# singforai/mini-marl

Hardware: AMD Instinct MI355X
Metric: agent-env-steps/sec (4096 envs x 8 agents per GPU, QMIX GRU-64 rollout step) (higher is better)
Workload: dtype f32 (agent forward: fp16x3-split MFMA emulating f32 products, f32 accumulate); 1 GPU; QMIX 8-agent gridworld rollout, 4096 envs/GPU, GRU-64 agents, chunk 10, PER; envs_per_gpu=4096, agents=8, obs_dim=47, f1=64, gru=64, chunk=10, per_capacity_chunks=65536, per_prefilled_chunks=65536, parallelism=env-shard x1

## Files before the change

mini-marl_amd/csrc/agent_fwd.hip:

```cpp
#include <algorithm>
#include <cstdlib>
#include <type_traits>

#include "common.h"
#include "env_dev.h"
#include "minimarl.h"
#include "qnet_geo.h"
#include "rollout_env.h"

namespace mm {

struct QFwdParams {
  mm_qfwd_io io;
  QnetGeo g;
  const float* packed;
  int E, N, D, A;
  int nblocks;
  int stagger;
  int dbg;
  int pad_;
};

__device__ __forceinline__ void load_frag(const float* __restrict__ base, int lane, float (&a)[16]) {
#pragma unroll
// ... 910 lines not shown
}

typedef _Float16 f16x8 __attribute__((ext_vector_type(8)));
typedef float f32x4 __attribute__((ext_vector_type(4)));
typedef float f32x2 __attribute__((ext_vector_type(2)));

__host__ __device__ __forceinline__ int kperm16(int j, int g) { return 16 * (j >> 2) + 4 * g + (j & 3); }

__device__ __forceinline__ f32x4 mfma16x16(const f16x8& a, const f16x8& b, f32x4 c) {
  return __builtin_amdgcn_mfma_f32_16x16x32_f16(a, b, c, 0, 0, 0);
}

struct KS {
  f16x8 h, l;
};
typedef _Float16 f16x2_ __attribute__((ext_vector_type(2)));
typedef float f32x2_ __attribute__((ext_vector_type(2)));
__device__ __forceinline__ void split8(const float (&x)[8], KS& t, int lo_pairs = 4) {
  uint32_t hw[4], lw[4];
#pragma unroll
  for (int j = 0; j < 4; ++j) {
    const f32x2_ v = {x[2 * j], x[2 * j + 1]};
    hw[j] = __builtin_bit_cast(uint32_t, __builtin_convertvector(v, f16x2_));
    uint32_t lo;
    if (j >= lo_pairs) {
      lw[j] = 0u;
    } else {
      asm("v_fma_mixlo_f16 %0, %1, -1.0, %2 op_sel_hi:[1,0,0]" : "=v"(lo) : "v"(hw[j]), "v"(v.x));
      asm("v_fma_mixhi_f16 %0, %1, -1.0, %2 op_sel:[1,0,0] op_sel_hi:[1,0,0]" : "+v"(lo) : "v"(hw[j]), "v"(v.y));
      lw[j] = lo;
    }
  }
  t.h = __builtin_bit_cast(f16x8, hw);
  t.l = __builtin_bit_cast(f16x8, lw);
}
__device__ __forceinline__ void split_pair(const f32x4& a, const f32x4& b, KS& t) {
  float x[8];
#pragma unroll
  for (int r = 0; r < 4; ++r) {
    x[r] = a[r];
    x[4 + r] = b[r];
  }
  split8(x, t);
}
__device__ __forceinline__ void mm16(const float* __restrict__ blk, int q, const KS& x, int lane, f32x4& acc) {
  const f16x8 ah = *reinterpret_cast<const f16x8*>(blk + (q * 2) * 256 + lane * 4);
  const f16x8 al = *reinterpret_cast<const f16x8*>(blk + (q * 2 + 1) * 256 + lane * 4);
  acc = mfma16x16(al, x.h, acc);
  acc = mfma16x16(ah, x.l, acc);
  acc = mfma16x16(ah, x.h, acc);
}
__device__ __forceinline__ void mm16_x16(const float* __restrict__ blk, int q, const KS& x, int lane, f32x4& acc) {
  const f16x8 ah = *reinterpret_cast<const f16x8*>(blk + (q * 2) * 256 + lane * 4);
  const f16x8 al = *reinterpret_cast<const f16x8*>(blk + (q * 2 + 1) * 256 + lane * 4);
  acc = mfma16x16(al, x.h, acc);
  acc = mfma16x16(ah, x.h, acc);
}
struct Frag {
  f16x8 h, l;
};
__device__ __forceinline__ Frag ldfrag(const float* __restrict__ blk, int q, int lane) {
  Frag f;
  f.h = *reinterpret_cast<const f16x8*>(blk + (q * 2) * 256 + lane * 4);
  f.l = *reinterpret_cast<const f16x8*>(blk + (q * 2 + 1) * 256 + lane * 4);
  return f;
}
__device__ __forceinline__ void mmf(const Frag& a, const KS& x, f32x4& acc) {
  acc = mfma16x16(a.l, x.h, acc);
  acc = mfma16x16(a.h, x.l, acc);
  acc = mfma16x16(a.h, x.h, acc);
}
__device__ __forceinline__ f32x4 bias4(const float* __restrict__ b, int t, int g) {
  return *reinterpret_cast<const f32x4*>(b + 16 * t + 4 * g);
}
__device__ __forceinline__ void load_obs_ks(const float* orow, int kb, int D, float (&x)[8]) {
  const int g = (threadIdx.x & 63) >> 4;
#pragma unroll
  for (int j = 0; j < 8; ++j) {
    const int k = kb * 32 + kperm16(j, g);
    x[j] = (orow && k < D) ? orow[k] : 0.0f;
  }
}

template <int AT>
__device__ __forceinline__ int q_epilogue16(const QFwdParams& p, int agent, int e, bool valid,
                                            const f32x4 (&qa)[AT], float eps, uint64_t ctr, int64_t out_off = 0,
                                            const uint64_t* rng_in = nullptr) {
  const int g = (threadIdx.x & 63) >> 4;
  const mm_qfwd_io& io = p.io;
  if (valid && io.q_out) {
    float* qrow = io.q_out + (int64_t)e * io.q_se + (int64_t)agent * io.q_sa;
#pragma unroll
    for (int t = 0; t < AT; ++t)
#pragma unroll
      for (int r = 0; r < 4; ++r) {
        const int row = 16 * t + 4 * g + r;
        if (row < p.A) qrow[row] = qa[t][r];
      }
  }
  if (io.mode == MM_Q_NONE) return 0;
  float best = -INFINITY;
  int bi = 0x7fffffff;
#pragma unroll
  for (int t = 0; t < AT; ++t)
#pragma unroll
    for (int r = 0; r < 4; ++r) {
      const int row = 16 * t + 4 * g + r;
      const float v = qa[t][r];
      if (row < p.A && (v > best || (v == best && row < bi))) {
        best = v;
        bi = row;
      }
    }
#pragma unroll
  for (int o = 16; o <= 32; o <<= 1) {
    const float ob = __shfl_xor(best, o);
    const int oi = __shfl_xor(bi, o);
    if (ob > best || (ob == best && oi < bi)) {
      best = ob;
      bi = oi;
    }
  }
  int act = bi;
  if (io.mode == MM_Q_ACT) {
    if (!io.u && !io.rand_act) {
      const bool ra_lane = (g & 1) != 0;
      const uint64_t sd = ra_lane ? io.seed ^ 0x5bd1e995ull : io.seed;
      const uint64_t r = rng_in ? rng_draw_inner(sd, ctr, *rng_in)
                                : rng_draw(sd, ctr, (uint64_t)e, ra_lane ? (uint64_t)agent : 0xFFFFFFFFull);
      const float uu = rng_uniform(r);
      const uint32_t Au = (uint32_t)p.A;
      const int ra = (int)rng_mod_small_u(r, Au, 0xFFFFFFFFu / Au, (0xFFFFFFFFu % Au + 1u) % Au);
      const float uo = __shfl_xor(uu, 16);
      const int rao = __shfl_xor(ra, 16);
      if ((ra_lane ? uo : uu) <= eps) act = ra_lane ? ra : rao;
    } else {
      float u;
      if (io.u) {
        u = valid ? io.u[e] : 1.0f;
      } else {
        u = rng_uniform(rng_draw(io.seed, ctr, (uint64_t)e, 0xFFFFFFFFull));
      }
      if (u <= eps) {
        if (io.rand_act) {
          act = valid ? io.rand_act[(int64_t)e * p.N + agent] : 0;
        } else {
          act = (int)(rng_draw(io.seed ^ 0x5bd1e995ull, ctr, (uint64_t)e, (uint64_t)agent) % (uint64_t)p.A);
        }
      }
    }
  } else if (io.mode == MM_Q_GATHER) {
    act = valid ? io.act_in[(int64_t)e * io.act_se + agent] : 0;
  }
  float mine = 0.0f;
#pragma unroll
  for (int t = 0; t < AT; ++t)
#pragma unroll
    for (int r = 0; r < 4; ++r)
      if (16 * t + 4 * g + r == act) mine = qa[t][r];
  mine += __shfl_xor(mine, 16);
  mine += __shfl_xor(mine, 32);
  const float qsel = (io.mode == MM_Q_MAX) ? best : mine;
  if (valid && g == 0) {
    const int64_t o = out_off + (int64_t)e * p.N + agent;
    if (io.act_out && io.mode == MM_Q_ACT) io.act_out[o] = act;
    if (io.qsel_out) io.qsel_out[o] = qsel;
  }
  return act;
}

template <int F1, int G, int H, int AB, class OL>
__device__ __forceinline__ int agent_q_fwd_body_h3(const QFwdParams& p, int agent, int e,
                                                    const float* __restrict__ W, const OL& ol,
                                                    float (&xn)[8], const f32x4 (&h0)[H / 16], float eps,
                                                    uint64_t ctr, int64_t out_off = 0, int x16_from_kb = 1 << 30,
                                                    f32x4 (*h1_keep)[H / 16] = nullptr, bool store_h = true,
                                                    const uint64_t* rng_in = nullptr) {
  using CG = QnetCGeo<F1, G, H, AB>;
  constexpr int T1 = F1 / 16, T2 = G / 16, TH = H / 16, AT = (AB * 32 + 15) / 16;
  constexpr int RB1 = F1 / 32, RB2 = G / 32, HB = H / 32;
  const int lane = threadIdx.x & 63;
  const int g = lane >> 4;
  const bool valid = e < p.E;
  const mm_qfwd_io& io = p.io;
  const int ATr = (p.A + 15) / 16;
  constexpr int NWB = (CG::off_b1 + 15359) / 15360;
  auto lds_opaque = [](const float* q) {
    auto l = (const __attribute__((address_space(3))) float*)q;
    asm volatile("" : "+v"(l));
    return (const float*)l;
  };
  const float* WL[NWB];
#pragma unroll
  for (int k = 0; k < NWB; ++k) WL[k] = lds_opaque(W + 15360 * k + lane * 4);
  const float* WBias = lds_opaque(W + CG::off_b1 + 4 * g);
  auto wblk = [&](int off) { return WL[off / 15360] + (off % 15360); };
  auto wbias = [&](int off, int t) { return *reinterpret_cast<const f32x4*>(WBias + (off - CG::off_b1) + 16 * t); };
  auto mmb = [&](int off, int q, const KS& x, f32x4& acc) {
    const f16x8 ah = *reinterpret_cast<const f16x8*>(wblk(off) + (q * 2) * 256);
    const f16x8 al = *reinterpret_cast<const f16x8*>(wblk(off) + (q * 2 + 1) * 256);
    acc = mfma16x16(al, x.h, acc);
    acc = mfma16x16(ah, x.l, acc);
    acc = mfma16x16(ah, x.h, acc);
  };
  auto frag = [&](int off, int q) {
    Frag f;
    f.h = *reinterpret_cast<const f16x8*>(wblk(off) + (q * 2) * 256);
    f.l = *reinterpret_cast<const f16x8*>(wblk(off) + (q * 2 + 1) * 256);
    return f;
  };

  f32x4 x1[T1];
#pragma unroll
  for (int t = 0; t < T1; ++t) x1[t] = wbias(CG::off_b1, t);
  for (int kb = 0; kb < p.g.KD; ++kb) {
    KS ob;
    split8(xn, ob, kb >= x16_from_kb ? 0 : (x16_from_kb == 1 ? 1 : 4));
    if (kb + 1 < p.g.KD) ol(kb + 1, xn);
    if (kb >= x16_from_kb) {
#pragma unroll
      for (int t = 0; t < T1; ++t)
        mm16_x16(W + CG::off_l1 + (int64_t)((t >> 1) * p.g.KD + kb) * 1024, t & 1, ob, lane, x1[t]);
    } else {
#pragma unroll
      for (int t = 0; t < T1; ++t)
        mm16(W + CG::off_l1 + (int64_t)((t >> 1) * p.g.KD + kb) * 1024, t & 1, ob, lane, x1[t]);
    }
  }
  KS x1s[RB1];
#pragma unroll
  for (int t = 0; t < T1; ++t)
#pragma unroll
    for (int r = 0; r < 4; ++r) x1[t][r] = relu_bits(x1[t][r]);
#pragma unroll
  for (int kb = 0; kb < RB1; ++kb) split_pair(x1[2 * kb], x1[2 * kb + 1], x1s[kb]);
  float* sv = (io.save && valid) ? io.save + ((int64_t)e * p.N + agent) * (F1 + G + 6 * H) : nullptr;
  if (sv) {
#pragma unroll
    for (int t = 0; t < T1; ++t)
#pragma unroll
      for (int r = 0; r < 4; ++r) sv[16 * t + 4 * g + r] = x1[t][r];
  }

  f32x4 x2[T2];
#pragma unroll
  for (int t = 0; t < T2; ++t) {
    x2[t] = wbias(CG::off_b2, t);
#pragma unroll
    for (int kb = 0; kb < RB1; ++kb) mmb(CG::off_l2 + ((t >> 1) * RB1 + kb) * 1024, t & 1, x1s[kb], x2[t]);
#pragma unroll
    for (int r = 0; r < 4; ++r) x2[t][r] = relu_bits(x2[t][r]);
    if (sv) {
#pragma unroll
      for (int r = 0; r < 4; ++r) sv[F1 + 16 * t + 4 * g + r] = x2[t][r];
    }
  }
  KS x2s[RB2];
#pragma unroll
  for (int kb = 0; kb < RB2; ++kb) split_pair(x2[2 * kb], x2[2 * kb + 1], x2s[kb]);

  KS h0s[HB];
#pragma unroll
  for (int kb = 0; kb < HB; ++kb) split_pair(h0[2 * kb], h0[2 * kb + 1], h0s[kb]);
  float* hop = (valid && io.h_out && store_h) ? io.h_out + (int64_t)e * io.hout_se + (int64_t)agent * io.hout_sa +
                                         (int64_t)(4 * g) * io.hout_sf
                                   : nullptr;
  f32x4 h1[TH];
#pragma unroll
  for (int t = 0; t < TH; ++t) {
    const int rb = t >> 1, q = t & 1;
    f32x4 ar = wbias(CG::off_brz, t);
    f32x4 az = wbias(CG::off_brz + H, t);
    f32x4 anx = wbias(CG::off_bin, t);
    f32x4 anh = wbias(CG::off_bhn, t);
    auto tri = [&](int base, int gstride, const KS& x, f32x4& a0, f32x4& a1, f32x4& a2) {
      const Frag f0 = frag(base, q);
      const Frag f1 = frag(base + gstride, q);
      const Frag f2 = frag(base + 2 * gstride, q);
      a0 = mfma16x16(f0.l, x.h, a0);
      a1 = mfma16x16(f1.l, x.h, a1);
      a2 = mfma16x16(f2.l, x.h, a2);
      a0 = mfma16x16(f0.h, x.l, a0);
      a1 = mfma16x16(f1.h, x.l, a1);
      a2 = mfma16x16(f2.h, x.l, a2);
      a0 = mfma16x16(f0.h, x.h, a0);
      a1 = mfma16x16(f1.h, x.h, a1);
      a2 = mfma16x16(f2.h, x.h, a2);
    };
#pragma unroll
    for (int kb = 0; kb < RB2; ++kb) tri(CG::off_ih + (rb * RB2 + kb) * 1024, HB * RB2 * 1024, x2s[kb], ar, az, anx);
#pragma unroll
    for (int kb = 0; kb < HB; ++kb) tri(CG::off_hh + (rb * HB + kb) * 1024, HB * HB * 1024, h0s[kb], ar, az, anh);
    float rrs[4], zs[4], ns[4];
#pragma unroll
    for (int rp = 0; rp < 4; rp += 2) {
      const f32x2 vr = {ar[rp], ar[rp + 1]}, vz = {az[rp], az[rp + 1]};
      const f32x2 vx = {anx[rp], anx[rp + 1]}, vh = {anh[rp], anh[rp + 1]}, v0 = {h0[t][rp], h0[t][rp + 1]};
      f32x2 er = vr * -1.4426950408889634f, ez = vz * -1.4426950408889634f;
      er.x = __builtin_amdgcn_exp2f(er.x);
      er.y = __builtin_amdgcn_exp2f(er.y);
      ez.x = __builtin_amdgcn_exp2f(ez.x);
      ez.y = __builtin_amdgcn_exp2f(ez.y);
      er = er + 1.0f;
      ez = ez + 1.0f;
      f32x2 rr, z;
      rr.x = __builtin_amdgcn_rcpf(er.x);
      rr.y = __builtin_amdgcn_rcpf(er.y);
      z.x = __builtin_amdgcn_rcpf(ez.x);
      z.y = __builtin_amdgcn_rcpf(ez.y);
      f32x2 en = (vx + rr * vh) * 2.8853900817779268f;
      en.x = __builtin_amdgcn_exp2f(en.x);
      en.y = __builtin_amdgcn_exp2f(en.y);
      en = en + 1.0f;
      f32x2 n;
      n.x = __builtin_amdgcn_rcpf(en.x);
      n.y = __builtin_amdgcn_rcpf(en.y);
      n = 1.0f - 2.0f * n;
      const f32x2 hn = n + z * (v0 - n);
      h1[t][rp] = hn.x;
      h1[t][rp + 1] = hn.y;
      rrs[rp] = rr.x;
      rrs[rp + 1] = rr.y;
      zs[rp] = z.x;
      zs[rp + 1] = z.y;
      ns[rp] = n.x;
      ns[rp + 1] = n.y;
    }
    if (sv) {
#pragma unroll
      for (int r = 0; r < 4; ++r) {
        float* o = sv + F1 + G + 16 * t + 4 * g + r;
        o[0] = h0[t][r];
        o[H] = rrs[r];
        o[2 * H] = zs[r];
        o[3 * H] = ns[r];
        o[4 * H] = anh[r];
        o[5 * H] = h1[t][r];
      }
    }
    if (hop) {
#pragma unroll
      for (int r = 0; r < 4; ++r) hop[(int64_t)(16 * t + r) * io.hout_sf] = h1[t][r];
    }
  }
  if (h1_keep) {
#pragma unroll
    for (int t = 0; t < TH; ++t) (*h1_keep)[t] = h1[t];
  }
  KS h1s[HB];
#pragma unroll
  for (int kb = 0; kb < HB; ++kb) split_pair(h1[2 * kb], h1[2 * kb + 1], h1s[kb]);

  f32x4 qa[AT];
#pragma unroll
  for (int t = 0; t < AT; ++t) {
    qa[t] = wbias(CG::off_bq, t);
    if (t < ATr) {
#pragma unroll
      for (int kb = 0; kb < HB; ++kb) mmb(CG::off_q + ((t >> 1) * HB + kb) * 1024, t & 1, h1s[kb], qa[t]);
    }
  }
  return q_epilogue16<AT>(p, agent, e, valid, qa, eps, ctr, out_off, rng_in);
}

__device__ __forceinline__ bool agent_range_guarded(const QFwdParams& p, int agent) {
  return reinterpret_cast<const int*>(p.packed + 2 * p.g.agent_stride * p.N)[agent] != 0;
}
__device__ __forceinline__ const float* agent_image_src(const QFwdParams& p, int agent, bool exact) {
  return p.packed + (exact ? 0 : (int64_t)p.N * p.g.agent_stride) + (int64_t)agent * p.g.agent_stride;
}
__device__ __forceinline__ void image_dma(const float* src, float* wsm, int nchunk, int first_wave, int n_waves) {
  const int wave = threadIdx.x >> 6, lane = threadIdx.x & 63;
  if (wave >= first_wave)
    for (int c = wave - first_wave; c < nchunk; c += n_waves) glds_dwordx4(src + c * 256 + lane * 4, wsm + c * 256);
}
template <int H>
__device__ __forceinline__ void load_h0(const mm_qfwd_io& io, int ec, int agent, int g, f32x4 (&h0)[H / 16]) {
  const float* hp = io.h_in + (int64_t)ec * io.hin_se + (int64_t)agent * io.hin_sa + (int64_t)(4 * g) * io.hin_sf;
#pragma unroll
  for (int t = 0; t < H / 16; ++t)
#pragma unroll
    for (int r = 0; r < 4; ++r) h0[t][r] = hp[(int64_t)(16 * t + r) * io.hin_sf];
}

template <int F1, int G, int H, int AB>
__global__ __launch_bounds__(1024, 1) void agent_q_fwd_h3_kernel(QFwdParams p0, QFwdParams p1) {
  extern __shared__ __attribute__((aligned(16))) float wsm[];
  const bool second = (int)blockIdx.x >= p0.nblocks;
  const QFwdParams* kargs = (const QFwdParams*)__builtin_amdgcn_kernarg_segment_ptr();
  static_assert(sizeof(QFwdParams) % 8 == 0, "kernarg layout");
  const QFwdParams& p = kargs[second ? 1 : 0];
  (void)p1;
  const int bid = second ? (int)blockIdx.x - p0.nblocks : (int)blockIdx.x;
  const int agent = bid % p.N, tile = bid / p.N;
  const int wave = threadIdx.x >> 6, lane = threadIdx.x & 63;
  if (agent_range_guarded(p, agent)) {
    const int e32 = tile * 256 + wave * 32 + (lane & 31);
    const float* src32 = agent_image_src(p, agent, true);
    const int nch = (int)(p.g.agent_stride >> 8);
    for (int c = wave; c < nch; c += 16) glds_dwordx4(src32 + c * 256 + lane * 4, wsm + c * 256);
    const float* orow32 = obs_row_ptr(p, agent, e32);
    float x32[16];
    load_obs_kblock(orow32, 0, p.D, x32);
    const bool zero_h = e32 >= p.E || (p.io.reset && p.io.reset[e32]);
    __syncthreads();
    if (wave < 8)
      agent_q_fwd_body<F1, G, H, AB>(p, agent, e32, wsm,
                                     [&](int kb, float (&x)[16]) { load_obs_kblock(orow32, kb, p.D, x); }, x32,
                                     zero_h);
    return;
  }
  const int e = tile * 256 + wave * 16 + (lane & 15);
  const int g = lane >> 4;
  const float* src = agent_image_src(p, agent, false);
  const int nchunk = (int)(p.g.agent_stride >> 8);
  for (int c = wave; c < nchunk; c += 16) glds_dwordx4(src + c * 256 + lane * 4, wsm + c * 256);
  const mm_qfwd_io& io = p.io;
  const int ec = min(e, p.E - 1);
  f32x4 h0[H / 16];
  if (io.h_in) {
    load_h0<H>(io, ec, agent, g, h0);
  } else {
#pragma unroll
    for (int t = 0; t < H / 16; ++t) h0[t] = f32x4{0.f, 0.f, 0.f, 0.f};
  }
  const bool reset = io.reset && io.reset[ec];
  const float* orow = obs_row_ptr(p, agent, e);
  float xn[8];
  load_obs_ks(orow, 0, p.D, xn);
  const float eps = (io.mode == MM_Q_ACT && io.eps_ptr) ? *io.eps_ptr : io.epsilon;
  const uint64_t ctr = (io.mode == MM_Q_ACT && io.counter_ptr) ? *io.counter_ptr : io.counter;
  if (e >= p.E || reset) {
#pragma unroll
    for (int t = 0; t < H / 16; ++t) h0[t] = f32x4{0.f, 0.f, 0.f, 0.f};
  }
  __syncthreads();
  if (wave >= 8)
    for (int i = 0; i < p.stagger; ++i) __builtin_amdgcn_s_sleep(8);
  agent_q_fwd_body_h3<F1, G, H, AB>(p, agent, e, wsm,
                                    [&](int kb, float (&x)[8]) { load_obs_ks(orow, kb, p.D, x); }, xn, h0, eps, ctr);
}

struct RollStep {
  EnvDev env;
  const int32_t* act;
// ... 348 lines not shown
  uint64_t ctr0, seq;
  float eps;
  int tile, agent, e0;
  bool second, writer;
};

template <int F1, int G, int H, int AB>
__device__ __forceinline__ ChunkCtx chunk_ctx(const QFwdParams* kargs) {
  const RollChunk& rc = *reinterpret_cast<const RollChunk*>(kargs + 2);
  const int nb = (int)gridDim.x, b = (int)blockIdx.x;
  const int lb = (nb % 8 == 0) ? (b % 8) * (nb / 8) + b / 8 : b;
  const int N = kargs[0].N;
  ChunkCtx cx;
  cx.tile = lb / (2 * N);
  const int role = lb % (2 * N);
  cx.second = role >= N;
  cx.agent = cx.second ? role - N : role;
  cx.writer = !cx.second && cx.agent == 0;
  cx.e0 = cx.tile * 256;
  const RollChunkLds lay = roll_chunk_lds(rc.env.R, rc.env.C, N);
  char* envl = reinterpret_cast<char*>(wsm_ptr()) + rc.lds_env;
  cx.stab = reinterpret_cast<float*>(envl + lay.stab);
  cx.sgrid = reinterpret_cast<uint32_t*>(envl + lay.sgrid);
  cx.spq = reinterpret_cast<uint16_t*>(envl + lay.spq);
  cx.ssa = reinterpret_cast<uint16_t*>(envl + lay.ssa);
  cx.sdone = reinterpret_cast<uint8_t*>(envl + lay.sdone);
  cx.shx = reinterpret_cast<uint8_t*>(envl + lay.shx);
  cx.sgrp = reinterpret_cast<uint32_t*>(envl + lay.sgrp);
  cx.ctr0 = *rc.counter;
  cx.seq = *rc.seq;
  cx.eps = cx.second ? *kargs[1].io.eps_ptr : 0.0f;
  return cx;
}

typedef __attribute__((address_space(3))) uint32_t lds_u32_t;
__device__ __forceinline__ void grp_arrive(uint32_t* ctr, int lane) {
  asm volatile("s_waitcnt lgkmcnt(0)" ::: "memory");
  if (lane == 0) __hip_atomic_fetch_add((lds_u32_t*)ctr, 1u, __ATOMIC_RELAXED, __HIP_MEMORY_SCOPE_WORKGROUP);
  asm volatile("" ::: "memory");
}
__device__ __forceinline__ void grp_wait(uint32_t* ctr, uint32_t target, uint32_t* err, int lane) {
  auto seen = [&]() {
    return __builtin_amdgcn_readfirstlane(
               __hip_atomic_load((lds_u32_t*)ctr, __ATOMIC_RELAXED, __HIP_MEMORY_SCOPE_WORKGROUP)) >= target;
  };
  if (!seen()) {
    const uint64_t tw = __builtin_amdgcn_s_memrealtime();
    while (true) {
      __builtin_amdgcn_s_sleep(1);
      if (seen()) break;
      if (__builtin_amdgcn_s_memrealtime() - tw > kHandoffTimeout) {
        if (lane == 0) atomicOr(err, 2u);
        break;
      }
    }
  }
  asm volatile("" ::: "memory");
}

#if MM_ROLL_DEBUG
#define MM_CSTAMP(k)                                                                                          \
  do {                                                                                                        \
    if (rc.trace && lane == 0 && i < 12 && second) {                                                          \
      const int gj = roll_group_of_wave(wave);                                                                \
      const int ws = wave == roll_group_dyn_wave(gj) ? 0 : (wave == 4 * gj + ((gj + 1) & 3) ? 1 : -1);         \
      const int64_t ix = (((((int64_t)cx.tile * N + agent) * 4 + gj) * 2 + ws) * 12 + i) * 4 + (k);           \
      if (ws >= 0 && ix < 60000) rc.trace[ix] = __builtin_amdgcn_s_memrealtime();                             \
    }                                                                                                         \
  } while (0)
#else
#define MM_CSTAMP(k) \
  do {               \
  } while (0)
#endif

template <int F1, int G, int H, int AB, bool EXACT>
__device__ __forceinline__ void roll_chunk_steps() {
  const QFwdParams* kargs0 = (const QFwdParams*)__builtin_amdgcn_kernarg_segment_ptr();
  const int nsteps = reinterpret_cast<const RollChunk*>(kargs0 + 2)->n;
  f32x4 hkeep[H / 16];
#pragma unroll
  for (int t = 0; t < H / 16; ++t) hkeep[t] = f32x4{0.f, 0.f, 0.f, 0.f};
  uint64_t rin = 0;
  if (!EXACT) {
    const ChunkCtx c0x = chunk_ctx<F1, G, H, AB>(kargs0);
    const int l0 = (int)threadIdx.x & 63;
    const int e_r = c0x.e0 + ((int)threadIdx.x >> 6) * 16 + (l0 & 15);
    rin = rng_inner((uint64_t)e_r, ((l0 >> 4) & 1) ? (uint64_t)c0x.agent : 0xFFFFFFFFull);
  }
  for (int i = 0; i < nsteps; ++i) {
  int tz = 0;
  asm volatile("" : "+s"(tz));
  const QFwdParams* kargs =
      (const QFwdParams*)((const __attribute__((address_space(4))) char*)__builtin_amdgcn_kernarg_segment_ptr() + tz);
  (void)kargs0;
  const int tx = (int)threadIdx.x + tz;
  const int wave = tx >> 6, lane = tx & 63;
  const ChunkCtx cx = chunk_ctx<F1, G, H, AB>(kargs);
  const QFwdParams& p = kargs[cx.second ? 1 : 0];
  const RollChunk& rc = *reinterpret_cast<const RollChunk*>(kargs + 2);
  const int CL = rc.CL;
  const EnvDev& ev = rc.env;
  const int N = p.N, D = p.D, R = ev.R, C = ev.C, E = p.E;
  const int64_t EN = (int64_t)E * N, nd = (int64_t)N * D;
  const mm_qfwd_io& io = p.io;
  const int tile = cx.tile, agent = cx.agent, e0 = cx.e0;
  const bool second = cx.second, writer = cx.writer;
  const int grp = roll_group_of_wave(wave);
  const bool dynw = EXACT ? tx < 256 : wave == roll_group_dyn_wave(grp);
  uint32_t* gc = cx.sgrp + kRollGroupCtrs * grp;
  const int le_d = EXACT ? tx : roll_group_env0(grp) + lane, de = e0 + le_d;
  const bool dvalid = dynw && de < E;
  uint32_t* rows = cx.sgrid + le_d * roll_gbw(R);
  const int le = wave * 16 + (lane & 15), e = e0 + le;
  const int l32 = wave * 32 + (lane & 31), e32 = e0 + l32;
    int c = rc.c0 + i, kset = rc.set0;
    uint32_t kcs = rc.c0 == 0 ? 1u : 0u;
    while (c >= CL) {
      c -= CL;
      kset = kset + 1 == rc.S ? 0 : kset + 1;
      ++kcs;
    }
    const int64_t* stg = rc.staging + (int64_t)kset * E;
    const int pos = rc.pos0 + i >= rc.RL ? rc.pos0 + i - rc.RL : rc.pos0 + i;
    const int posn = pos + 1 == rc.RL ? 0 : pos + 1;
    const uint64_t ctr = cx.ctr0 + (uint64_t)i;
    const int cur = i & 1, prv = cur ^ 1;
    MM_CSTAMP(0);
    if (!EXACT &&
        __builtin_amdgcn_readfirstlane(wave) == roll_group_dyn_wave(__builtin_amdgcn_readfirstlane(grp)))
      __builtin_amdgcn_s_setprio(3);
    uint32_t aq[2] = {0u, 0u};
    if (i > 0) {
      if constexpr (!EXACT) {
        if (dynw) {
          const int w0 = roll_group_word0(grp);
          const uint64_t* hs = rc.hx + ((int64_t)tile * rc.hxl + i) * N * 32 + w0;
          uint32_t* hl = reinterpret_cast<uint32_t*>(cx.shx) + w0;
          const uint32_t tag = (uint32_t)cx.seq + 1u;
          constexpr int NQ = (kRollMaxN * 8 + 63) / 64;
          const int nw = N * 8;
          int wo[NQ];
          uint32_t got = 0u;
#pragma unroll
          for (int q = 0; q < NQ; ++q) {
            const int ix = q * 64 + lane;
            wo[q] = (ix >> 3) * 32 + (ix & 7);
            if (ix >= nw) got |= 1u << q;
          }
          const uint32_t need = (1u << NQ) - 1u;
          const uint64_t tw = __builtin_amdgcn_s_memrealtime();
          while (true) {
            uint64_t w[NQ];
#pragma unroll
            for (int q = 0; q < NQ; ++q)
              if (!((got >> q) & 1u)) w[q] = __hip_atomic_load(hs + wo[q], __ATOMIC_RELAXED, __HIP_MEMORY_SCOPE_AGENT);
#pragma unroll
            for (int q = 0; q < NQ; ++q)
              if (!((got >> q) & 1u) && (uint32_t)(w[q] >> 32) == tag) {
                hl[wo[q]] = (uint32_t)w[q];
                got |= 1u << q;
              }
            if (__all(got == need)) break;
            __builtin_amdgcn_s_sleep(1);
            if (__builtin_amdgcn_s_memrealtime() - tw > kHandoffTimeout) {
              if (lane == 0) atomicOr(rc.err, 2u);
// ... 96 lines not shown
      const int st = (int)cx.ssa[le_d] + 1;
      int apples = cx.ssa[256 + le_d];
      float* rout = rc.rew + (int64_t)pos * EN + (int64_t)de * N;
#pragma unroll
      for (int k = 0; k < kRollMaxN; ++k) {
        if (k < N) {
          const uint32_t w = pq[0] & 0xFFFFu;
          const int a = (int)(aq[0] & 15u);
#pragma unroll
          for (int j = 0; j < kRollMaxN / 2 - 1; ++j) pq[j] = __builtin_amdgcn_alignbit(pq[j + 1], pq[j], 16);
          pq[kRollMaxN / 2 - 1] >>= 16;
          aq[0] = __builtin_amdgcn_alignbit(aq[1], aq[0], 4);
          aq[1] >>= 4;
          const RollMove mv = roll_agent_step(w, a, k, rows, R, C, ev.step_cost);
          apples -= mv.ate ? 1 : 0;
          cx.spq[le_d * N + k] = (uint16_t)mv.w;
          if (writer) rout[k] = mv.rew;
        }
      }
      const bool dn = st >= ev.max_steps || apples == 0;
      cx.ssa[le_d] = (uint16_t)st;
      cx.ssa[256 + le_d] = (uint16_t)apples;
      cx.sdone[cur * 256 + le_d] = dn ? 1 : 0;
      if (writer) {
        rc.done[(int64_t)pos * E + de] = dn ? 1 : 0;
        rc.cur_row[de] = dn ? -1 : myrow;
      }
    }
    if constexpr (EXACT) {
      __syncthreads();
    } else {
      if (dynw)
        grp_arrive(gc + 1, lane);
      else
        grp_wait(gc + 1, (uint32_t)i + 1u, rc.err, lane);
    }
    MM_CSTAMP(2);
    const int64_t off = (int64_t)(second ? posn : pos) * EN;
    const int64_t nxt_off = (int64_t)(c + 1) * nd;
    if constexpr (EXACT) {
      const int hh = lane >> 5;
      if (wave < 8) {
        const bool ok32 = e32 < E;
        const bool r32 = !second && ok32 && cx.sdone[prv * 256 + l32];
        const bool bd = second && ok32 && cx.sdone[cur * 256 + l32];
        float* dst = (!second && srow >= 0) ? rc.store_obs + srow * rc.row_stride + nxt_off + (int64_t)agent * D : nullptr;
        const int ls = ok32 ? l32 : 0;
        const int rc32 = cx.spq[ls * N + agent] & 0xFF;
        const uint64_t wd32 = roll_obs_word(cx.sgrid + ls * roll_gbw(R), R, rc32 >> 4, rc32 & 15);
        const float cr32 = cx.stab[rc32 >> 4], cc32 = cx.stab[R + (rc32 & 15)];
        auto ol32 = [&](int kb, float (&x)[16]) {
#pragma unroll
          for (int q = 0; q < 4; ++q) {
            const int f0 = kb * 32 + 8 * q + 4 * hh;
            roll_feat4(wd32, f0, cr32, cc32, x + 4 * q);
            if (bd || !ok32)
#pragma unroll
              for (int j = 0; j < 4; ++j) x[4 * q + j] = (ok32 && f0 + j < D) ? ev.reset_obs[agent * D + f0 + j] : 0.0f;
            if (dst) roll_store4(dst, f0, D, x + 4 * q);
          }
        };
        float x32[16];
        ol32(0, x32);
        const int a = agent_q_fwd_body<F1, G, H, AB>(p, agent, ok32 ? e32 : E, wsm_ptr() + tz, ol32, x32,
                                                     !ok32 || r32 || bd, true, cx.eps, ctr, off);
        if (second && hh == 0 && ok32) cx.shx[l32] = (uint8_t)a;
      }
    } else {
      const int ec = min(e, E - 1);
      const int g = lane >> 4;
      f32x4 h0[H / 16];
      if (i == 0) {
        load_h0<H>(io, ec, agent, g, h0);
      } else {
#pragma unroll
        for (int t = 0; t < H / 16; ++t) h0[t] = hkeep[t];
      }
      const bool rt = !second && e < E && cx.sdone[prv * 256 + le];
      const bool bd = second && e < E && cx.sdone[cur * 256 + le];
      if (e >= E || rt || bd) {
#pragma unroll
        for (int t = 0; t < H / 16; ++t) h0[t] = f32x4{0.f, 0.f, 0.f, 0.f};
      }
      float* dst = (!second && srow >= 0) ? rc.store_obs + srow * rc.row_stride + nxt_off + (int64_t)agent * D : nullptr;
      const int ls = e < E ? le : 0;
      const int rcw = cx.spq[ls * N + agent] & 0xFF;
      const uint64_t wd = roll_obs_word_g(cx.sgrid + ls * roll_gbw(R), R, rcw >> 4, rcw & 15, g);
      const float cr = cx.stab[rcw >> 4], cc = cx.stab[R + (rcw & 15)];
      grp_arrive(gc + 0, lane);
      auto ol = [&](int kb, float (&x)[8]) {
#pragma unroll
        for (int q = 0; q < 2; ++q) {
          const int f0 = kb * 32 + 16 * q + 4 * g;
          roll_feat4(wd, f0, cr, cc, x + 4 * q);
          if (bd || e >= E)
#pragma unroll
            for (int j = 0; j < 4; ++j) x[4 * q + j] = (e < E && f0 + j < D) ? ev.reset_obs[agent * D + f0 + j] : 0.0f;
          if (dst) roll_store4(dst, f0, D, x + 4 * q);
        }
      };
      float xn[8];
      ol(0, xn);
      switch (__builtin_amdgcn_readfirstlane((grp + i) & 3)) {
        case 0: __builtin_amdgcn_s_setprio(0); break;
        case 1: __builtin_amdgcn_s_setprio(1); break;
        case 2: __builtin_amdgcn_s_setprio(2); break;
        default: __builtin_amdgcn_s_setprio(3); break;
      }
      const int a = agent_q_fwd_body_h3<F1, G, H, AB>(p, agent, e, wsm_ptr() + tz, ol, xn, h0, cx.eps, ctr, off, 1,
                                                      &hkeep, i + 1 == nsteps, &rin);
      if (second && i + 1 < rc.n) {
        uint32_t v = ((uint32_t)a & 15u) << (4 * (lane & 7));
        v |= __shfl_xor(v, 1);
        v |= __shfl_xor(v, 2);
        v |= __shfl_xor(v, 4);
        if (lane == 0 || lane == 8) {
          uint64_t* hd = rc.hx + (((int64_t)tile * rc.hxl + i + 1) * N + agent) * 32 + wave * 2 + (lane >> 3);
          __hip_atomic_store(hd, ((uint64_t)((uint32_t)cx.seq + 1u) << 32) | v, __ATOMIC_RELAXED,
                             __HIP_MEMORY_SCOPE_AGENT);
        }
      }
    }
    MM_CSTAMP(3);
    if (EXACT && second && i + 1 < rc.n) {
      __syncthreads();
      if (wave == 0 && lane < 32) {
        const uint2 b = reinterpret_cast<const uint2*>(cx.shx)[lane];
        uint64_t* hd = rc.hx + (((int64_t)tile * rc.hxl + i + 1) * N + agent) * 32 + lane;
        __hip_atomic_store(hd, ((uint64_t)((uint32_t)cx.seq + 1u) << 32) | nib_pack4(b.x) | (nib_pack4(b.y) << 16),
                           __ATOMIC_RELAXED, __HIP_MEMORY_SCOPE_AGENT);
      }
    }
  }
  if constexpr (!EXACT) __syncthreads();
}

template <int F1, int G, int H, int AB>
__global__ __launch_bounds__(1024, 1) void rollout_chunk_kernel(QFwdParams p0, QFwdParams p1, RollChunk rc_) {
  float* wsm = wsm_ptr();
  const QFwdParams* kargs = (const QFwdParams*)__builtin_amdgcn_kernarg_segment_ptr();
  const RollChunk& rc = *reinterpret_cast<const RollChunk*>(kargs + 2);
  (void)p0;
  (void)p1;
  (void)rc_;
  const int N = kargs[0].N;
  const ChunkCtx cx = chunk_ctx<F1, G, H, AB>(kargs);
  const int nb = (int)gridDim.x;
  const QFwdParams& p = kargs[cx.second ? 1 : 0];
  const EnvDev& ev = rc.env;
  const int R = ev.R, C = ev.C, RC = R * C, E = p.E;
  const int agent = cx.agent, e0 = cx.e0;
  const bool exact = agent_range_guarded(p, agent);
  const int par = *rc.envpar;

  image_dma(agent_image_src(p, agent, exact), wsm, (int)(p.g.agent_stride >> 8), 0, 16);
  if (threadIdx.x >= 256 && threadIdx.x < 256 + R + C) {
    const int i = threadIdx.x - 256;
    cx.stab[i] = i < R ? ev.rtab[i] : ev.ctab[i - R];
  }
  const int le_d = threadIdx.x, de = e0 + le_d;
  const bool dvalid = threadIdx.x < 256 && de < E;
  if (dvalid) {
    const int32_t* pw = (par ? ev.pos_alt : ev.pos) + (int64_t)de * N;
    const uint4* gin = reinterpret_cast<const uint4*>((par ? ev.grid_alt : ev.grid) + (int64_t)de * RC);
    uint32_t* rows = cx.sgrid + le_d * roll_gbw(R);
    cx.ssa[le_d] = (uint16_t)(par ? ev.steps_alt : ev.steps)[de];
    cx.ssa[256 + le_d] = (uint16_t)(par ? ev.apples_alt : ev.apples)[de];
    for (int k = 0; k < N; ++k) cx.spq[le_d * N + k] = (uint16_t)pos16(pw[k]);
    roll_unpack_rows(gin, rows, R);
    cx.sdone[256 + le_d] = rc.done_prev[de];
    if (cx.writer) {
      int ks = rc.set0;
      for (int k = 0; k < rc.S && k * rc.CL < rc.c0 + rc.n; ++k) {
        roll_row_ok(rc.staging[(int64_t)ks * E + de], rc.n_rows, rc.err);
        ks = ks + 1 == rc.S ? 0 : ks + 1;
      }
    }
  } else if (threadIdx.x < 256) {
    cx.sdone[256 + le_d] = 0;
  }
  if (threadIdx.x >= 512 && threadIdx.x < 512 + kRollGroups * kRollGroupCtrs) cx.sgrp[threadIdx.x - 512] = 0u;
  __syncthreads();

#if MM_ROLL_DEBUG
  uint64_t* clk = (rc.trace && threadIdx.x == 0) ? rc.trace + 60000 + 4 * (int)blockIdx.x : nullptr;
  if (clk) {
    clk[0] = __builtin_amdgcn_s_memtime();
    clk[1] = __builtin_amdgcn_s_memrealtime();
  }
#endif
  if (exact)
    roll_chunk_steps<F1, G, H, AB, true>();
  else
    roll_chunk_steps<F1, G, H, AB, false>();
#if MM_ROLL_DEBUG
  if (clk) {
    clk[2] = __builtin_amdgcn_s_memtime();
    clk[3] = __builtin_amdgcn_s_memrealtime();
// ... 653 lines not shown
  rc = make_params(d, packed_b, io_b, n_envs, &p1);
  if (rc) return rc;
  RollStep rs;
  rs.env = env->d;
  rs.act = x->act;
  rs.store_obs = x->store_obs;
  rs.row_stride = x->row_stride;
  rs.next_off = (int64_t)x->slot * nd;
  rs.staging = x->staging;
  rs.cur_row = x->cur_row;
  rs.rew = x->rew;
  rs.done = x->done;
  rs.counter = x->counter;
  rs.td = TdFuse{};
  if (x->td_on) {
    MM_REQUIRE(x->td_rew && x->td_done && x->td_qsel && x->td_maxq && x->td_act && x->chunk_td && x->store_act &&
                   x->store_rew && x->store_done, "rollout_step: null TD argument");
    MM_REQUIRE(x->td_slot >= 0 && x->td_slot < x->chunk_len, "rollout_step: bad TD slot");
    rs.td = TdFuse{x->td_rew, x->td_done, x->td_qsel, x->td_maxq, x->td_act, x->chunk_td, x->store_act,
                   x->store_rew, x->store_done, x->staging, nullptr, x->gamma, x->td_slot, x->chunk_len, 1};
  }
  rs.par = x->state_in;
#if MM_ROLL_DEBUG
  rs.trace = debug_trace_buffer("MM_ROLL_TRACE");
#else
  rs.trace = nullptr;
#endif
  MM_REQUIRE(x->n_rows >= 1 && x->n_rows < (1ll << 40), "rollout_step: n_rows must be the chunk store's row count");
  rs.n_rows = x->n_rows;
  rs.err = reinterpret_cast<uint32_t*>(x->err);
  rs.begin = x->begin ? 1 : 0;
  rs.lds_env = (int)roll_region(env->d, p0.g);
  if (with_qnet_shape(d, &rc, [&](auto F1, auto G, auto H, auto AB) {
        return launch_roll<F1, G, H, AB>(p0, p1, rs, sm, s);
      }))
    return rc;
  set_error("rollout_step: unsupported (F1,G,H)");
  return MM_EINVAL;
}

size_t rollout_chunk_lds(const mm_env* env, const mm_qnet_dims* d, int64_t n_envs) {
  if (rollout_step_lds(env, d, n_envs) == 0) return 0;
  const EnvDev& ev = env->d;
  QnetGeo g;
  QnetOffsets o;
  if (qnet_geometry(d, &g, &o)) return 0;
  const size_t img = ((size_t)g.agent_stride * 4 + 15) & ~size_t(15);
  const size_t sm = img + (size_t)roll_chunk_lds(ev.R, ev.C, ev.N).total;
  if (sm > 160 * 1024) return 0;
  int dev = 0, cus = 0;
  if (hipGetDevice(&dev) != hipSuccess || hipDeviceGetAttribute(&cus, hipDeviceAttributeMultiprocessorCount, dev) !=
                                              hipSuccess) {
    (void)hipGetLastError();
    return 0;
  }
  const int64_t nb = 2 * (int64_t)ev.N * ((n_envs + 255) / 256);
  return nb <= cus ? sm : 0;
}

int rollout_chunk(mm_env* env, const mm_qnet_dims* d, const float* packed_t, const mm_qfwd_io* io_t,
                  const float* packed_b, const mm_qfwd_io* io_b, int64_t n_envs, const mm_rollout_chunk_io* x,
                  hipStream_t s) {
  MM_REQUIRE(env && d && x && io_t && io_b, "rollout_chunk: null argument");
  const size_t sm = rollout_chunk_lds(env, d, n_envs);
  MM_REQUIRE(sm > 0, "rollout_chunk: configuration not supported (mm_rollout_chunk_supported)");
  const EnvDev& ev = env->d;
  MM_REQUIRE(x->store_obs && x->staging && x->cur_row && x->act0 && x->done_prev && x->rew && x->done && x->counter &&
                 x->ctl && x->handoff, "rollout_chunk: null buffer");
  MM_REQUIRE(x->chunk_len >= 1 && x->chunk_len <= 4096 && x->c0 >= 0 && x->c0 < x->chunk_len && x->n_steps >= 1,
             "rollout_chunk: bad chunk position / step count");
  MM_REQUIRE(x->n_sets >= 1 && x->n_sets <= 64 && x->set0 >= 0 && x->set0 < x->n_sets &&
                 x->c0 + x->n_steps <= (int64_t)x->n_sets * x->chunk_len,
             "rollout_chunk: the launch's steps span more chunks than staging sets (%d)", x->n_sets);
  MM_REQUIRE(x->ring_len >= 2 && x->ring_pos >= 0 && x->ring_pos < x->ring_len && x->n_steps < x->ring_len,
             "rollout_chunk: the rings must hold the launch's steps plus the next step's actions (n_steps < ring_len)");
  MM_REQUIRE(x->handoff_len >= x->n_steps, "rollout_chunk: handoff_len < n_steps");
  MM_REQUIRE(x->n_rows >= 1 && x->n_rows < (1ll << 40), "rollout_chunk: n_rows must be the chunk store's row count");
  MM_REQUIRE(io_t->mode == MM_Q_MAX && io_b->mode == MM_Q_ACT, "rollout_chunk: target io must be MAX, behavior io ACT");
  MM_REQUIRE(io_t->h_in && io_b->h_in && io_t->h_in == io_t->h_out && io_b->h_in == io_b->h_out,
             "rollout_chunk: hidden states required, updated in place");
  MM_REQUIRE(io_b->eps_ptr && io_b->act_out && io_b->qsel_out && io_t->qsel_out,
             "rollout_chunk: behavior eps_ptr / act_out / qsel_out and target qsel_out required");
  MM_REQUIRE(io_b->reset == nullptr && io_t->reset == nullptr, "rollout_chunk: reset flags come from the env (pass NULL)");
  const int64_t nd = (int64_t)d->n_agents * d->obs_dim;
  MM_REQUIRE(x->row_stride >= (x->chunk_len + 1) * nd, "rollout_chunk: row stride too small");
  QFwdParams p0, p1;
  mm_qfwd_io i0 = *io_t, i1 = *io_b;
  i0.obs = i1.obs = ev.reset_obs;
  int rc = make_params(d, packed_t, &i0, n_envs, &p0);
  if (rc) return rc;
  rc = make_params(d, packed_b, &i1, n_envs, &p1);
  if (rc) return rc;
  const int tiles = (int)((n_envs + 255) / 256);
  p0.nblocks = p1.nblocks = tiles * d->n_agents;
  RollChunk r;
  r.env = ev;
  r.store_obs = x->store_obs;
  r.row_stride = x->row_stride;
  r.staging = x->staging;
  r.cur_row = x->cur_row;
  r.n_rows = x->n_rows;
  r.act0 = x->act0;
  r.done_prev = x->done_prev;
  r.rew = x->rew;
  r.done = x->done;
  r.counter = reinterpret_cast<uint64_t*>(x->counter);
  r.seq = reinterpret_cast<uint64_t*>(x->ctl);
  r.envpar = reinterpret_cast<int32_t*>(x->ctl + 1);
  r.ticket = reinterpret_cast<uint32_t*>(x->ctl + 2);
  r.hx = reinterpret_cast<uint64_t*>(x->handoff);
  r.err = reinterpret_cast<uint32_t*>(x->err);
#if MM_ROLL_DEBUG
  r.trace = debug_trace_buffer("MM_ROLL_TRACE");
#else
  r.trace = nullptr;
#endif
  r.c0 = x->c0;
  r.n = x->n_steps;
  r.CL = x->chunk_len;
  r.S = x->n_sets;
  r.set0 = x->set0;
  r.RL = x->ring_len;
  r.pos0 = x->ring_pos;
  r.hxl = x->handoff_len;
  QnetGeo g;
  QnetOffsets o;
  qnet_geometry(d, &g, &o);
  r.lds_env = (int)(((size_t)g.agent_stride * 4 + 15) & ~size_t(15));
  const int nb = 2 * tiles * d->n_agents;
  if (with_qnet_shape(d, &rc, [&](auto F1, auto G, auto H, auto AB) {
        return launch_chunk<F1, G, H, AB>(p0, p1, r, nb, sm, s);
      }))
    return rc;
  set_error("rollout_chunk: unsupported (F1,G,H)");
  return MM_EINVAL;
}

}
```

mini-marl_amd/csrc/common.h:

```cpp
#pragma once
#include <hip/hip_runtime.h>
#include <stdint.h>

#define MM_OK 0
#define MM_EINVAL (-22)
#define MM_EHIP (-5)
#define MM_ENOMEM (-12)

namespace mm {

void set_error(const char* fmt, ...);

typedef float f32x16 __attribute__((ext_vector_type(16)));

__host__ __device__ __forceinline__ int kperm(int s, int h) { return (s & 3) + 8 * (s >> 2) + 4 * h; }

__device__ __forceinline__ f32x16 mfma32(float a, float b, f32x16 c) {
  return __builtin_amdgcn_mfma_f32_32x32x2f32(a, b, c, 0, 0, 0);
}

__device__ __forceinline__ float sigmoidf_(float x) {
  return __builtin_amdgcn_rcpf(1.0f + __builtin_amdgcn_exp2f(x * -1.4426950408889634f));
}
__device__ __forceinline__ float tanhf_(float x) {
  return 1.0f - 2.0f * __builtin_amdgcn_rcpf(1.0f + __builtin_amdgcn_exp2f(x * 2.8853900817779268f));
}

__device__ __forceinline__ uint64_t mix64(uint64_t z) {
  z += 0x9E3779B97F4A7C15ull;
  z = (z ^ (z >> 30)) * 0xBF58476D1CE4E5B9ull;
  z = (z ^ (z >> 27)) * 0x94D049BB133111EBull;
  return z ^ (z >> 31);
}
__device__ __forceinline__ uint64_t rng_draw(uint64_t seed, uint64_t counter, uint64_t a, uint64_t b) {
  return mix64(seed ^ mix64(counter * 0xD1B54A32D192ED03ull ^ mix64(a * 0x8CB92BA72F3D8DD7ull + b)));
}
__device__ __forceinline__ uint64_t rng_inner(uint64_t a, uint64_t b) { return mix64(a * 0x8CB92BA72F3D8DD7ull + b); }
__device__ __forceinline__ uint64_t rng_draw_inner(uint64_t seed, uint64_t counter, uint64_t inner) {
  return mix64(seed ^ mix64(counter * 0xD1B54A32D192ED03ull ^ inner));
}
__device__ __forceinline__ uint32_t umod_small(uint32_t x, uint32_t m, uint32_t minv) {
  uint32_t r = x - __umulhi(x, minv) * m;
  r = r >= m ? r - m : r;
  return r >= m ? r - m : r;
}
__device__ __forceinline__ float rollout_td(float sr, float sq, float st, float d, float gamma) {
  const float boot = __fmul_rn(__fmul_rn(1.0f - d, gamma), st);
  return fabsf(__fsub_rn(__fadd_rn(sr, boot), sq));
}
__device__ __forceinline__ float rng_uniform(uint64_t r) { return (float)(r >> 40) * (1.0f / 16777216.0f); }
__device__ __forceinline__ uint32_t rng_mod_small(uint64_t r, uint32_t m) {
  const uint32_t p32 = (0xFFFFFFFFu % m + 1u) % m;
  return ((uint32_t)(r >> 32) % m * p32 + (uint32_t)r % m) % m;
}
__device__ __forceinline__ uint32_t rng_mod_small_u(uint64_t r, uint32_t m, uint32_t minv, uint32_t p32) {
  return umod_small(umod_small((uint32_t)(r >> 32), m, minv) * p32 + umod_small((uint32_t)r, m, minv), m, minv);
}
__device__ __forceinline__ float relu_bits(float x) {
  return __int_as_float(max(__float_as_int(x), 0));
}

uint64_t* debug_trace_buffer(const char* env_name);

typedef __attribute__((address_space(3))) void lds_void_t;
__device__ __forceinline__ void glds_dword(const void* g, float* lds_base) {
  __builtin_amdgcn_global_load_lds(g, (lds_void_t*)lds_base, 4, 0, 0);
}
template <typename A>
__device__ __forceinline__ void glds_gather(float* dst, int n, A addr) {
  const int lane = threadIdx.x & 63, nw = blockDim.x >> 6;
  for (int c0 = (int)(threadIdx.x >> 6) * 64; c0 < n; c0 += nw * 64)
    if (c0 + lane < n) glds_dword(addr(c0 + lane), dst + c0);
}
template <typename A>
__device__ __forceinline__ void glds_rows(float* dst, int rows, int rowlen, int ld, A addr) {
  const int lane = threadIdx.x & 63, nw = blockDim.x >> 6;
  const int pr = (rowlen + 63) >> 6;
  for (int q = (int)(threadIdx.x >> 6); q < rows * pr; q += nw) {
    const int r = q / pr, c0 = (q - r * pr) * 64;
    if (c0 + lane < rowlen) glds_dword(addr(r, c0 + lane), dst + r * ld + c0);
  }
}

__device__ __forceinline__ void glds_dwordx4(const void* g, float* lds_base) {
  __builtin_amdgcn_global_load_lds(g, (lds_void_t*)lds_base, 16, 0, 0);
}
template <typename S>
__device__ __forceinline__ void glds_rows16(float* dst, int rows, int rowlen, int ld, S src) {
  const int lane = threadIdx.x & 63, nw = blockDim.x >> 6;
  const int pr = (rowlen + 255) >> 8;
  for (int q = (int)(threadIdx.x >> 6); q < rows * pr; q += nw) {
    const int r = q / pr, c0 = (q - r * pr) * 256;
    if (c0 + 4 * lane < rowlen) glds_dwordx4(src(r) + c0 + 4 * lane, dst + r * ld + c0);
  }
}

template <typename A>
__device__ __forceinline__ void glds16_gather(float* dst, int n4, A addr) {
  const int lane = threadIdx.x & 63, nw = blockDim.x >> 6;
  for (int c0 = (int)(threadIdx.x >> 6) * 64; c0 < n4; c0 += nw * 64)
    if (c0 + lane < n4) glds_dwordx4(addr(c0 + lane), dst + 4 * c0);
}

__device__ __forceinline__ void lds_sync() { asm volatile("s_waitcnt lgkmcnt(0)\n\ts_barrier" ::: "memory"); }

template <int K>
__device__ __forceinline__ float dot_seq(const float* w, const float* x, float acc) {
#pragma unroll
  for (int k = 0; k < K; ++k) acc += w[k] * x[k];
  return acc;
}
__device__ __forceinline__ float dot_seq_n(const float* w, const float* x, int K, float acc) {
  if (K == 64) return dot_seq<64>(w, x, acc);
  if (K == 32) return dot_seq<32>(w, x, acc);
  for (int k = 0; k < K; ++k) acc += w[k] * x[k];
  return acc;
}

struct TdFuse {
  const float* rew;
  const uint8_t* done;
  const float* q_taken;
// ... 41 lines not shown
```

Measured before the change: 1.714 billion agent-env-steps/s.

## Specialize chunk rollout step: carry split hidden state, single Q tile, lane-swap epilogue

Adds a compile-time StepChunk policy for the rollout chunk loop. It carries the already-split fp16 hidden state across steps instead of re-splitting h0, computes only one 16-row Q tile (n_actions <= 16), and drops the save/q_out paths. It also replaces the shuffle-based argmax and action reductions with permlane16/32 swaps and DPP, and batches RNG draws for two steps into one, carrying the decision to the odd step. This adds host-side requirements (n_actions <= 16, no q_out/save/u/rand_act) and changes which RNG lanes produce the draws, which may alter the random stream.

```diff
diff --git a/mini-marl_amd/csrc/agent_fwd.hip b/mini-marl_amd/csrc/agent_fwd.hip
--- a/mini-marl_amd/csrc/agent_fwd.hip
+++ b/mini-marl_amd/csrc/agent_fwd.hip
@@ -1016,10 +1016,100 @@
   }
 }
 
-template <int AT>
+struct StepGeneric {
+  static constexpr bool kGeneric = true;
+};
+struct StepChunk {
+  static constexpr bool kGeneric = false;
+};
+
+struct LanePair {
+  uint32_t lo, hi;
+};
+__device__ __forceinline__ LanePair lane_pair16(uint32_t v) {
+  const auto x = __builtin_amdgcn_permlane16_swap(v, v, false, false);
+  return LanePair{x[0], x[1]};
+}
+__device__ __forceinline__ LanePair lane_pair32(uint32_t v) {
+  const auto x = __builtin_amdgcn_permlane32_swap(v, v, false, false);
+  return LanePair{x[0], x[1]};
+}
+
+template <int MODE>
+__device__ __forceinline__ int q_epilogue16_chunk(const QFwdParams& p, int agent, int e, bool valid, const f32x4& q0,
+                                                  float eps, uint64_t ctr, int64_t out_off, const uint64_t* rng_in,
+                                                  bool odd_step, int& carry) {
+  const int g = (threadIdx.x & 63) >> 4;
+  const mm_qfwd_io& io = p.io;
+  float best = -INFINITY;
+  int bi = 0x7fffffff;
+#pragma unroll
+  for (int r = 0; r < 4; ++r) {
+    const int row = 4 * g + r;
+    const float v = q0[r];
+    if (row < p.A && (v > best || (v == best && row < bi))) {
+      best = v;
+      bi = row;
+    }
+  }
+  auto better = [&](const LanePair& v, const LanePair& ix) {
+    const float fa = __uint_as_float(v.lo), fb = __uint_as_float(v.hi);
+    const int ia = (int)ix.lo, ib = (int)ix.hi;
+    const bool tb = fb > fa || (fb == fa && ib < ia);
+    best = tb ? fb : fa;
+    bi = tb ? ib : ia;
+  };
+  better(lane_pair16(__float_as_uint(best)), lane_pair16((uint32_t)bi));
+  better(lane_pair32(__float_as_uint(best)), lane_pair32((uint32_t)bi));
+  static_assert(MODE == MM_Q_ACT || MODE == MM_Q_MAX, "chunk step epilogue: behavior (ACT) or target (MAX)");
+  if constexpr (MODE == MM_Q_MAX) {
+    if (valid && g == 0) io.qsel_out[out_off + (int64_t)e * p.N + agent] = best;
+    return bi;
+  } else {
+    int dec;
+    if (!odd_step) {
+      const bool ra_lane = (g & 1) != 0;
+      const uint64_t sd = ra_lane ? io.seed ^ 0x5bd1e995ull : io.seed;
+      const uint64_t r = rng_draw_premul(sd, (g & 2) ? rng_counter_mul(ctr + 1) : rng_counter_mul(ctr), *rng_in);
+      const float uu = rng_uniform(r);
+      const uint32_t Au = (uint32_t)p.A;
+      const uint32_t ra = rng_mod_small_u(r, Au, 0xFFFFFFFFu / Au, (0xFFFFFFFFu % Au + 1u) % Au);
+      const float u = __uint_as_float(lane_pair16(__float_as_uint(uu)).lo);
+      const int d = u <= eps ? (int)lane_pair16(ra).hi : -1;
+      const LanePair dd = lane_pair32((uint32_t)d);
+      dec = (int)dd.lo;
+      carry = (int)dd.hi;
+    } else {
+      dec = carry;
+    }
+    const int act = dec >= 0 ? dec : bi;
+    float mine = 0.0f;
+#pragma unroll
+    for (int r = 0; r < 4; ++r)
+      if (4 * g + r == act) mine = q0[r];
+    const LanePair m16 = lane_pair16(__float_as_uint(mine));
+    mine = __uint_as_float(m16.lo) + __uint_as_float(m16.hi);
+    const LanePair m32 = lane_pair32(__float_as_uint(mine));
+    mine = __uint_as_float(m32.lo) + __uint_as_float(m32.hi);
+    if (valid && g == 0) {
+      const int64_t o = out_off + (int64_t)e * p.N + agent;
+      io.act_out[o] = act;
+      io.qsel_out[o] = mine;
+    }
+    return act;
+  }
+}
+
+template <int AT, class POL = StepGeneric>
 __device__ __forceinline__ int q_epilogue16(const QFwdParams& p, int agent, int e, bool valid,
                                             const f32x4 (&qa)[AT], float eps, uint64_t ctr, int64_t out_off = 0,
-                                            const uint64_t* rng_in = nullptr) {
+                                            const uint64_t* rng_in = nullptr, bool odd_step = false,
+                                            int* carry = nullptr) {
+  if constexpr (!POL::kGeneric) {
+    if (p.io.mode == MM_Q_ACT)
+      return q_epilogue16_chunk<MM_Q_ACT>(p, agent, e, valid, qa[0], eps, ctr, out_off, rng_in, odd_step, *carry);
+    return q_epilogue16_chunk<MM_Q_MAX>(p, agent, e, valid, qa[0], eps, ctr, out_off, rng_in, odd_step, *carry);
+  }
   const int g = (threadIdx.x & 63) >> 4;
   const mm_qfwd_io& io = p.io;
   if (valid && io.q_out) {
@@ -1103,15 +1193,17 @@
   return act;
 }
 
-template <int F1, int G, int H, int AB, class OL>
+template <int F1, int G, int H, int AB, class OL, class POL = StepGeneric>
 __device__ __forceinline__ int agent_q_fwd_body_h3(const QFwdParams& p, int agent, int e,
                                                     const float* __restrict__ W, const OL& ol,
                                                     float (&xn)[8], const f32x4 (&h0)[H / 16], float eps,
                                                     uint64_t ctr, int64_t out_off = 0, int x16_from_kb = 1 << 30,
                                                     f32x4 (*h1_keep)[H / 16] = nullptr, bool store_h = true,
-                                                    const uint64_t* rng_in = nullptr) {
+                                                    const uint64_t* rng_in = nullptr, bool odd_step = false,
+                                                    int* carry = nullptr, KS (*hs_carry)[H / 32] = nullptr) {
   using CG = QnetCGeo<F1, G, H, AB>;
   constexpr int T1 = F1 / 16, T2 = G / 16, TH = H / 16, AT = (AB * 32 + 15) / 16;
+  constexpr int QT = POL::kGeneric ? AT : 1;
   constexpr int RB1 = F1 / 32, RB2 = G / 32, HB = H / 32;
   const int lane = threadIdx.x & 63;
   const int g = lane >> 4;
@@ -1168,7 +1260,9 @@
     for (int r = 0; r < 4; ++r) x1[t][r] = relu_bits(x1[t][r]);
 #pragma unroll
   for (int kb = 0; kb < RB1; ++kb) split_pair(x1[2 * kb], x1[2 * kb + 1], x1s[kb]);
-  float* sv = (io.save && valid) ? io.save + ((int64_t)e * p.N + agent) * (F1 + G + 6 * H) : nullptr;
+  float* sv = nullptr;
+  if constexpr (POL::kGeneric)
+    sv = (io.save && valid) ? io.save + ((int64_t)e * p.N + agent) * (F1 + G + 6 * H) : nullptr;
   if (sv) {
 #pragma unroll
     for (int t = 0; t < T1; ++t)
@@ -1194,11 +1288,16 @@
   for (int kb = 0; kb < RB2; ++kb) split_pair(x2[2 * kb], x2[2 * kb + 1], x2s[kb]);
 
   KS h0s[HB];
-#pragma unroll
-  for (int kb = 0; kb < HB; ++kb) split_pair(h0[2 * kb], h0[2 * kb + 1], h0s[kb]);
-  float* hop = (valid && io.h_out && store_h) ? io.h_out + (int64_t)e * io.hout_se + (int64_t)agent * io.hout_sa +
-                                         (int64_t)(4 * g) * io.hout_sf
-                                   : nullptr;
+  if constexpr (!POL::kGeneric) {
+#pragma unroll
+    for (int kb = 0; kb < HB; ++kb) h0s[kb] = (*hs_carry)[kb];
+  } else {
+#pragma unroll
+    for (int kb = 0; kb < HB; ++kb) split_pair(h0[2 * kb], h0[2 * kb + 1], h0s[kb]);
+  }
+  float* hop = (valid && (!POL::kGeneric || io.h_out) && store_h)
+                   ? io.h_out + (int64_t)e * io.hout_se + (int64_t)agent * io.hout_sa + (int64_t)(4 * g) * io.hout_sf
+                   : nullptr;
   f32x4 h1[TH];
 #pragma unroll
   for (int t = 0; t < TH; ++t) {
@@ -1284,17 +1383,21 @@
   KS h1s[HB];
 #pragma unroll
   for (int kb = 0; kb < HB; ++kb) split_pair(h1[2 * kb], h1[2 * kb + 1], h1s[kb]);
-
-  f32x4 qa[AT];
-#pragma unroll
-  for (int t = 0; t < AT; ++t) {
+  if constexpr (!POL::kGeneric) {
+#pragma unroll
+    for (int kb = 0; kb < HB; ++kb) (*hs_carry)[kb] = h1s[kb];
+  }
+
+  f32x4 qa[QT];
+#pragma unroll
+  for (int t = 0; t < QT; ++t) {
     qa[t] = wbias(CG::off_bq, t);
-    if (t < ATr) {
+    if (!POL::kGeneric || t < ATr) {
 #pragma unroll
       for (int kb = 0; kb < HB; ++kb) mmb(CG::off_q + ((t >> 1) * HB + kb) * 1024, t & 1, h1s[kb], qa[t]);
     }
   }
-  return q_epilogue16<AT>(p, agent, e, valid, qa, eps, ctr, out_off, rng_in);
+  return q_epilogue16<QT, POL>(p, agent, e, valid, qa, eps, ctr, out_off, rng_in, odd_step, carry);
 }
 
 __device__ __forceinline__ bool agent_range_guarded(const QFwdParams& p, int agent) {
@@ -1809,6 +1912,8 @@
 #pragma unroll
   for (int t = 0; t < H / 16; ++t) hkeep[t] = f32x4{0.f, 0.f, 0.f, 0.f};
   uint64_t rin = 0;
+  KS hsk[H / 32] = {};
+  int dcarry = -1;
   if (!EXACT) {
     const ChunkCtx c0x = chunk_ctx<F1, G, H, AB>(kargs0);
     const int l0 = (int)threadIdx.x & 63;
@@ -2071,6 +2176,13 @@
 #pragma unroll
         for (int t = 0; t < H / 16; ++t) h0[t] = f32x4{0.f, 0.f, 0.f, 0.f};
       }
+      if (i == 0) {
+#pragma unroll
+        for (int kb = 0; kb < H / 32; ++kb) split_pair(h0[2 * kb], h0[2 * kb + 1], hsk[kb]);
+      } else if (e >= E || rt || bd) {
+#pragma unroll
+        for (int kb = 0; kb < H / 32; ++kb) hsk[kb] = KS{};
+      }
       float* dst = (!second && srow >= 0) ? rc.store_obs + srow * rc.row_stride + nxt_off + (int64_t)agent * D : nullptr;
       const int ls = e < E ? le : 0;
       const int rcw = cx.spq[ls * N + agent] & 0xFF;
@@ -2096,13 +2208,14 @@
         case 2: __builtin_amdgcn_s_setprio(2); break;
         default: __builtin_amdgcn_s_setprio(3); break;
       }
-      const int a = agent_q_fwd_body_h3<F1, G, H, AB>(p, agent, e, wsm_ptr() + tz, ol, xn, h0, cx.eps, ctr, off, 1,
-                                                      &hkeep, i + 1 == nsteps, &rin);
+      const int a = agent_q_fwd_body_h3<F1, G, H, AB, decltype(ol), StepChunk>(
+          p, agent, e, wsm_ptr() + tz, ol, xn, h0, cx.eps, ctr, off, 1, &hkeep, i + 1 == nsteps, &rin, (i & 1) != 0,
+          &dcarry, &hsk);
       if (second && i + 1 < rc.n) {
         uint32_t v = ((uint32_t)a & 15u) << (4 * (lane & 7));
-        v |= __shfl_xor(v, 1);
-        v |= __shfl_xor(v, 2);
-        v |= __shfl_xor(v, 4);
+        v |= (uint32_t)__builtin_amdgcn_update_dpp(0, (int)v, 0xB1, 0xF, 0xF, false);
+        v |= (uint32_t)__builtin_amdgcn_update_dpp(0, (int)v, 0x4E, 0xF, 0xF, false);
+        v |= (uint32_t)__builtin_amdgcn_update_dpp(0, (int)v, 0x141, 0xF, 0xF, false);
         if (lane == 0 || lane == 8) {
           uint64_t* hd = rc.hx + (((int64_t)tile * rc.hxl + i + 1) * N + agent) * 32 + wave * 2 + (lane >> 3);
           __hip_atomic_store(hd, ((uint64_t)((uint32_t)cx.seq + 1u) << 32) | v, __ATOMIC_RELAXED,
@@ -2922,6 +3035,9 @@
   MM_REQUIRE(io_b->eps_ptr && io_b->act_out && io_b->qsel_out && io_t->qsel_out,
              "rollout_chunk: behavior eps_ptr / act_out / qsel_out and target qsel_out required");
   MM_REQUIRE(io_b->reset == nullptr && io_t->reset == nullptr, "rollout_chunk: reset flags come from the env (pass NULL)");
+  MM_REQUIRE(d->n_actions <= 16, "rollout_chunk: the hand-off words carry 4-bit actions (n_actions <= 16)");
+  MM_REQUIRE(!io_b->u && !io_b->rand_act && !io_b->save && !io_t->save && !io_b->q_out && !io_t->q_out,
+             "rollout_chunk: device draws only, no q_out / save (the step loop's compile-time policy)");
   const int64_t nd = (int64_t)d->n_agents * d->obs_dim;
   MM_REQUIRE(x->row_stride >= (x->chunk_len + 1) * nd, "rollout_chunk: row stride too small");
   QFwdParams p0, p1;
diff --git a/mini-marl_amd/csrc/common.h b/mini-marl_amd/csrc/common.h
--- a/mini-marl_amd/csrc/common.h
+++ b/mini-marl_amd/csrc/common.h
@@ -38,6 +38,10 @@
 __device__ __forceinline__ uint64_t rng_inner(uint64_t a, uint64_t b) { return mix64(a * 0x8CB92BA72F3D8DD7ull + b); }
 __device__ __forceinline__ uint64_t rng_draw_inner(uint64_t seed, uint64_t counter, uint64_t inner) {
   return mix64(seed ^ mix64(counter * 0xD1B54A32D192ED03ull ^ inner));
+}
+__device__ __forceinline__ uint64_t rng_counter_mul(uint64_t counter) { return counter * 0xD1B54A32D192ED03ull; }
+__device__ __forceinline__ uint64_t rng_draw_premul(uint64_t seed, uint64_t cmul, uint64_t inner) {
+  return mix64(seed ^ mix64(cmul ^ inner));
 }
 __device__ __forceinline__ uint32_t umod_small(uint32_t x, uint32_t m, uint32_t minv) {
   uint32_t r = x - __umulhi(x, minv) * m;
```

Result: faster. 1.784 billion agent-env-steps/s (median of 6 runs) (+4.1%).
